# mlelarge/graph_neural_net

Hardware: AMD Instinct MI355X
Metric: graph-pairs/sec FGNN fwd+bwd, N=50 regular pairs (higher is better)
Workload: dtype f32

## Files before the change

graph_neural_net_amd/_lib.py:

```python
import ctypes as C
import os

import torch

_HERE = os.path.dirname(os.path.abspath(__file__))
LIB_PATH = os.environ.get('FGNN_LIB') or os.path.join(_HERE, 'libfgnn_hip.so')

FGNN_H = 32
FGNN_TILE = 32
FGNN_MAX_DEPTH = 3
FGNN_RANGE_WG = 256
FGNN_LSAP_MAX_N = 2048
FGNN_SCORE_SPLIT = 4

c_float_p = C.c_void_p


class Slab(C.Structure):
    _fields_ = [('ptr', C.c_void_p), ('gstride', C.c_longlong), ('ldp', C.c_longlong), ('C', C.c_int),
                ('nrm', C.c_void_p), ('beta', C.c_void_p)]


class MlpFwdArgs(C.Structure):
    _fields_ = [('G', C.c_int), ('N', C.c_int), ('depth', C.c_int), ('nmlp', C.c_int),
# ... 34 lines not shown
                ('dxb', C.c_void_p), ('dxb_gstride', C.c_longlong), ('dxb_ld', C.c_longlong),
                ('accumulate_dx', C.c_int), ('accumulate_dxb', C.c_int),
                ('wpart', C.c_void_p)]


class Mlp64PackJob(C.Structure):
    _fields_ = [('W', C.c_void_p * 3), ('bias', C.c_void_p * 3), ('cin', C.c_int), ('packed', C.c_void_p)]


class MlpBwdArgs(C.Structure):
    _fields_ = [('G', C.c_int), ('N', C.c_int), ('depth', C.c_int),
                ('nvalid', C.c_void_p),
                ('a', Slab), ('b', Slab),
                ('W', C.c_void_p * FGNN_MAX_DEPTH),
                ('bias', C.c_void_p * FGNN_MAX_DEPTH),
                ('dy', C.c_void_p), ('dgstride', C.c_longlong), ('ldd', C.c_longlong),
                ('z', C.c_void_p), ('zgstride', C.c_longlong), ('ldz', C.c_longlong),
                ('coef', C.c_void_p), ('s12', C.c_void_p), ('znrm', C.c_void_p),
                ('dxa', C.c_void_p), ('dxa_gstride', C.c_longlong), ('dxa_ld', C.c_longlong),
                ('dxb', C.c_void_p), ('dxb_gstride', C.c_longlong), ('dxb_ld', C.c_longlong),
                ('accumulate_a', C.c_int), ('accumulate_b', C.c_int),
                ('wpart', C.c_void_p), ('s12part', C.c_void_p), ('packed', C.c_void_p),
                ('s12tiles', C.c_void_p), ('s12_out', C.c_void_p), ('xbits', C.c_void_p), ('xdeg', C.c_void_p),
                ('ranges', C.c_void_p), ('cu_share', C.c_int)]


class Slab16(C.Structure):
    _fields_ = [('ptr', C.c_void_p), ('gstride', C.c_longlong), ('ldp', C.c_longlong), ('C', C.c_int),
                ('nrm', C.c_void_p), ('beta', C.c_void_p)]


class MlpFwd16Args(C.Structure):
    _fields_ = [('G', C.c_int), ('N', C.c_int), ('ldr', C.c_int), ('depth', C.c_int), ('nmlp', C.c_int),
                ('nvalid', C.c_void_p),
                ('a', Slab16), ('b', Slab16),
                ('z', C.c_void_p * 2), ('ldz', C.c_longlong),
                ('part', C.c_void_p * 2), ('cnt', C.c_void_p), ('packed', C.c_void_p), ('ranges', C.c_void_p)]


class MlpBwd16Args(C.Structure):
    _fields_ = [('G', C.c_int), ('N', C.c_int), ('ldr', C.c_int), ('depth', C.c_int),
                ('nvalid', C.c_void_p),
                ('a', Slab16), ('b', Slab16),
                ('dy', C.c_void_p), ('dgstride', C.c_longlong), ('ldd', C.c_longlong),
                ('z', C.c_void_p), ('zgstride', C.c_longlong), ('ldz', C.c_longlong),
                ('coef', C.c_void_p),
                ('dxa', C.c_void_p), ('dxa_gstride', C.c_longlong), ('dxa_ld', C.c_longlong),
# ... 70 lines not shown
    'fgnn_chan_matmul_fwd_fin_ord': [C.POINTER(Slab), C.POINTER(Slab), _VP, _VP, _VP, _VP, _VP, _F, _VP, _I, _I, _VP, _LL, _LL, _VP, _I, _VP],
    'fgnn_colmax_fwd': [C.POINTER(Slab), _VP, _I, _I, _VP, _VP, _VP],
    'fgnn_colmax_fwd_fin_supported': [_I],
    'fgnn_colmax_fwd_fin': [C.POINTER(Slab), _VP, _VP, _VP, _F, _VP, _I, _I, _VP, _VP, _VP],
    'fgnn_score_ce_fwd': [_VP, _VP, _VP, _I, _I, _I, _VP, _VP, _VP, _VP],
    'fgnn_score_row_blocks': [_I, _I],
    'fgnn_score_ce_fwd_blocks': [_VP, _VP, _VP, _I, _I, _I, _I, _VP, _VP, _VP, _VP],
    'fgnn_score_ce_bwd': [_VP, _VP, _VP, _VP, _VP, _VP, _I, _I, _I, _VP, _VP, _VP],
    'fgnn_inv_node_count': [_VP, _I, _VP, _VP],
    'fgnn_score_bwd': [_VP, _VP, _VP, _VP, _I, _I, _I, _VP, _VP, _VP],
    'fgnn_ce_fwd': [_VP, _VP, _I, _I, _VP, _VP, _VP],
    'fgnn_ce_bwd': [_VP, _VP, _VP, _VP, _I, _I, _VP, _VP],
    'fgnn_colmax_bwd': [_VP, _VP, _VP, _I, _I, _I, _VP, _LL, _LL, C.POINTER(Slab), _VP, _VP],
    'fgnn_gn_bwd_stats': [_VP, _LL, _LL, _VP, _LL, _LL, _VP, _VP, _I, _I, _I, _VP, _VP],
    'fgnn_gn_bwd_coef': [_VP, _VP, _VP, _I, _I, _I, _VP, _VP, _VP, _VP],
    'fgnn_gn_bwd_coef_tiles': [_VP, _VP, _VP, _I, _I, _I, _VP, _VP, _VP],
    'fgnn_grad_finalize': [_VP, _I, _I, _I, _I, _VP],
    'fgnn_gn_bwd_apply': [_VP, _LL, _LL, _VP, _LL, _LL, _VP, _VP, _I, _I, _I, _VP, _LL, _LL, _VP],
    'fgnn_mlp_bwd': [C.POINTER(MlpBwdArgs), _VP],
    'fgnn_mlp_bwd_x3': [C.POINTER(MlpBwdArgs), _VP],
    'fgnn_mlp_bwd_pair': [C.POINTER(MlpBwdArgs), C.POINTER(MlpBwdArgs), _VP],
    'fgnn_mlp_bwd_t16': [C.POINTER(MlpBwdArgs), _VP],
    'fgnn_mlp_bwd_t16_supported': [C.POINTER(MlpBwdArgs)],
    'fgnn_mlp_bwd_pair_t16': [C.POINTER(MlpBwdArgs), C.POINTER(MlpBwdArgs), _VP],
    'fgnn_mlp_bwd_pair_x3': [C.POINTER(MlpBwdArgs), C.POINTER(MlpBwdArgs), _VP],
    'fgnn_block1_struct_supported': [_I, _I, _I],
    'fgnn_block1_struct_table_floats': [_I],
    'fgnn_block1_struct_ws_floats': [_I, _I],
    'fgnn_block1_struct_rows': [_I, _I],
    'fgnn_block1_struct_fwd': [_VP, _VP, _I, _I, _VP, _VP, _VP, _VP, _VP, C.c_float, _VP, _VP, _VP, _LL, _LL, _VP, _VP, _VP, _VP, _VP, _VP, _VP],
    'fgnn_block1_struct_bwd': [_VP, _VP, _I, _I, _VP, _VP, _VP, _VP, _VP, _VP, _VP, _VP, _LL, _LL, _VP, _VP, _VP, _VP, _VP, _VP],
    'fgnn_block1_struct_fwd_pack': [_VP, _VP, _I, _I, _VP, _VP, _VP, _VP, _VP, C.c_float, _VP, _VP, _VP, _LL, _LL, _VP, _VP, _VP, _VP, _VP, _VP, _VP, _I, _VP],
    'fgnn_block1_struct_fwd16_pack': [_VP, _VP, _I, _I, _I, _VP, _VP, _VP, _VP, _VP, C.c_float, _VP, _VP, _VP, _LL, _LL, _VP, _VP, _VP, _VP, _VP, _VP, _VP, _I, _VP],
    'fgnn_block1_struct_fwd16': [_VP, _VP, _I, _I, _I, _VP, _VP, _VP, _VP, _VP, C.c_float, _VP, _VP, _VP, _LL, _LL, _VP, _VP, _VP, _VP, _VP, _VP, _VP],
    'fgnn_block1_struct_bwd16': [_VP, _VP, _I, _I, _I, _VP, _VP, _VP, _VP, _VP, _VP, _VP, _VP, _LL, _LL, _VP, _VP, _VP, _VP, _VP, _VP],
    'fgnn_mlp_bwd_coef_tiles_supported': [_I, _I],
    'fgnn_mlp_param_count': [_I, _I],
    'fgnn_reduce_partials': [_VP, _I, _I, _VP, _VP],
    'fgnn_chan_matmul_bwd': [C.POINTER(Slab), C.POINTER(Slab), _VP, _LL, _LL, _VP, _I, _I, _VP, _VP, _LL, _LL, _VP, _VP, _VP],
    'fgnn_chan_matmul_bwd_ord': [C.POINTER(Slab), C.POINTER(Slab), _VP, _LL, _LL, _VP, _I, _I, _VP, _VP, _LL, _LL, _VP, _VP, _VP, _I, _VP],
    'fgnn_sum_scale': [_VP, _I, _I, _F, _VP, _VP],
    'fgnn_adam_step': [_VP, _VP, _VP, _VP, _I, C.c_double, C.c_double, C.c_double, C.c_double, _I, C.c_double, _VP],
    'fgnn_adam_step_dev': [_VP, _VP, _VP, _VP, _I, _VP, _VP, _VP],
    'fgnn_expand_adjacency': [_VP, _VP, _I, _I, _VP, _VP],
    'fgnn_pack_adjacency': [_VP, _VP, _I, _I, _VP, _VP, _VP],
    'fgnn_pack_adjacency_ld': [_VP, _VP, _I, _I, _I, _VP, _VP, _VP],
# ... 123 lines not shown
```

graph_neural_net_amd/csrc/mlp_bwd_t16.hip:

```cpp
#include "fgnn_t16.h"
#include "fgnn_pack.h"

namespace {

using namespace t16;

constexpr int BWD_WG = 256;
constexpr int NW = 8;

DEVI float4 coef_from_sums(const float4 n, const float2 sv, float nv) {
    const float m = nv * nv;
    float4 k;
    k.x = n.x;
    k.y = n.y;
    k.z = m > 0.f ? -n.y * sv.y * n.w / m : 0.f;
    k.w = m > 0.f ? -n.y * sv.x / m : 0.f;
    return k;
}
DEVI int graph_nv(const rsrc_t &rnv, bool ragged, int g, int N) {
    const int v = __builtin_amdgcn_raw_buffer_load_b32(rnv, g * 4, 0, 0);
    return __builtin_amdgcn_readfirstlane(ragged ? v : N);
}

template <int CB>
struct Layout16 {
    static constexpr int DEPTH = 3;
    static constexpr PkBwd PK = pk_bwd(32, CB, DEPTH);
    static constexpr int OFF_W0A = PK.off_w1a, OFF_W0B = PK.off_w1b, OFF_W1 = PK.off_wh, OFF_WT1 = PK.off_wt, OFF_WT2 = PK.off_wt + 16;
    static constexpr int OFF_WT0A = PK.off_wt0a, OFF_WT0B = PK.off_wt0b;
    static constexpr int BIAS_F = PK.bias_f;
    static constexpr int WEIGHT_F = pk_pad_floats(PK.floats);
    static constexpr int NSLOT = 5;
    static constexpr int CIN = 32 + CB;
    static constexpr int PCOUNT = 32 * CIN + 32 + (DEPTH - 1) * (32 * 32 + 32);
    static constexpr int TILE_OFF = WEIGHT_F;
    static constexpr int REC_OFF = TILE_OFF + NW * NSLOT * TILE_F;
    static constexpr int WGK_OFF = REC_OFF + NW * 256;
    static constexpr int LIVE_OFF = WGK_OFF + FGNN_BWD_COEF_GRAPHS * 128;
    static constexpr int MAIN_F = LIVE_OFF + LIVE_LIST_CAP + NW;
    static constexpr int RED_F = NW * PCOUNT;
    static constexpr int LDS_F = MAIN_F > RED_F ? MAIN_F : RED_F;
};

template <int CB, bool PKD, bool SKIP, bool DXB>
__global__ __launch_bounds__(64 * NW, 2) void mlp_bwd_t16_kernel(const fgnn_mlp_bwd_args A, const int tpg, const int total_tiles) {
    extern __shared__ __attribute__((aligned(16))) float smem[];
    using L = Layout16<CB>;
    constexpr bool NB = CB == 32;
    const int lane = threadIdx.x & 63, wv = __builtin_amdgcn_readfirstlane(threadIdx.x >> 6);
    const int px = lane & 15, q = lane >> 4;
    const int P2 = A.N * A.N, hpg = 2 * tpg;
    const View va = make_view(A.a.ptr, A.a.gstride, A.a.ldp, A.G);
    const View vb = make_view(A.b.ptr, A.b.gstride, A.b.ldp, A.G);
    PackedSrc ps = {};
    if constexpr (PKD) ps = make_packed_src(A.xbits, A.xdeg, A.G, A.N);
    const View vdy = make_view(A.dy, A.dgstride, A.ldd, A.G);
    const View vz = make_view(A.z, A.zgstride, A.ldz, A.G);
    const View vdxa = make_view(A.dxa, A.dxa_gstride, A.dxa_ld, A.G);
    const View vdxb = make_view(A.dxb, A.dxb_gstride, A.dxb_ld, A.G);

    float *wl = smem;
    float *my = smem + L::TILE_OFF + wv * (L::NSLOT * TILE_F);
    float *XA = my, *XB = my + TILE_F, *S0 = my + 2 * TILE_F, *S1 = my + 3 * TILE_F, *S2 = my + 4 * TILE_F;
    const int lane_base = tile_lane_base(px, q);

    f32x4 dW0a[4], dW0b[4], dW1[4], dW2[4];
    float db0[2] = {0.f, 0.f}, db1[2] = {0.f, 0.f}, db2[2] = {0.f, 0.f}, dbx[2] = {0.f, 0.f};
#pragma unroll
    for (int k = 0; k < 4; ++k) dW0a[k] = dW0b[k] = dW1[k] = dW2[k] = zero4();

    const int nwg = gridDim.x;
    const int qq = total_tiles / nwg, rem = total_tiles % nwg;
    int T0 = blockIdx.x * qq + ((int)blockIdx.x < rem ? (int)blockIdx.x : rem);
    int T1 = T0 + qq + ((int)blockIdx.x < rem ? 1 : 0);
    if constexpr (SKIP) {
        T0 = A.ranges[blockIdx.x];
        T1 = A.ranges[blockIdx.x + 1];
    }
    const int H0 = 2 * T0, H1 = 2 * T1;
// ... 46 lines not shown
            while (h < H1) {
                const int g = h / hpg, hh = h - g * hpg;
                if (hh * 16 < P2) break;
                h += NW;
            }
            return __builtin_amdgcn_readfirstlane(h);
        }
    };

    pk_glds<NW>(smem, A.packed, L::WEIGHT_F, wv, lane);

    float mean[8], av[8], beta[8], kx[8], ky[8], kz[8], kw[8];
#pragma unroll
    for (int s = 0; s < 8; ++s) {
        mean[s] = 0.f;
        av[s] = 1.f;
        beta[s] = (NB && A.b.nrm && A.b.beta) ? A.b.beta[chan_s(s) + chan_q(q)] : 0.f;
        kx[s] = ky[s] = kz[s] = kw[s] = 0.f;
    }
    float4 *rec = reinterpret_cast<float4 *>(smem + L::REC_OFF) + wv * 64;
    auto fetch_records = [&](int g, int nv) {
        if (lane < 32) {
            float4 k4;
            if (from_tiles) k4 = wgK[(g - g0) * 32 + lane];
            else if (A.coef) k4 = reinterpret_cast<const float4 *>(A.coef)[(long long)g * FGNN_H + lane];
            else {
                const float4 n = reinterpret_cast<const float4 *>(A.znrm)[(long long)g * FGNN_H + lane];
                const float2 sv = reinterpret_cast<const float2 *>(A.s12)[(long long)g * FGNN_H + lane];
                k4 = coef_from_sums(n, sv, (float)nv);
            }
            rec[lane] = k4;
            if (NB && A.b.nrm) rec[32 + lane] = reinterpret_cast<const float4 *>(A.b.nrm)[(long long)g * A.b.C + lane];
        }
    };
    auto read_records = [&]() {
#pragma unroll
        for (int s = 0; s < 8; ++s) {
            const float4 k4 = rec[chan_s(s) + chan_q(q)];
            kx[s] = k4.x;
            ky[s] = k4.y;
            kz[s] = k4.z;
            kw[s] = k4.w;
            if (NB && A.b.nrm) {
                const float4 n = rec[32 + chan_s(s) + chan_q(q)];
                mean[s] = n.x;
                av[s] = n.y;
            }
        }
    };

    constexpr int NXB = CB == 32 ? 8 : 1;
    float xa[8], xb[NXB], dyr[8], zr[8];
    auto load_x = [&](int h) {
        const bool act = h < H1;
        const int g = __builtin_amdgcn_readfirstlane(act ? h / hpg : 0);
        const int p = (act ? h - g * hpg : 0) * 16 + px;
        const bool inb = act && p < P2;
        load8(xa, va, lane_voff(va, q, p, inb), g * va.gs4);
        if constexpr (CB == 32) {
            load8(xb, vb, lane_voff(vb, q, p, inb), g * vb.gs4);
        } else if constexpr (PKD) {
            int i, jj;
            row_col(p, A.N, rcpN, i, jj);
            const int ob = (inb && q == 0) ? (i * ps.words + (jj >> 5)) * 4 : OOB_OFF;
            const int od = (inb && q == 1 && i == jj) ? i * 4 : OOB_OFF;
            const unsigned w = (unsigned)__builtin_amdgcn_raw_buffer_load_b32(ps.bits, ob, g * ps.N * ps.words * 4, 0);
            const float d = __builtin_bit_cast(float, __builtin_amdgcn_raw_buffer_load_b32(ps.deg, od, g * ps.N * 4, 0));
            xb[0] = q == 0 ? (((w >> (jj & 31)) & 1u) ? 1.f : 0.f) : d;
        } else {
            xb[0] = buf_load(vb, (inb && q < 2) ? q * vb.ld4 + 4 * p : OOB_OFF, g * vb.gs4);
        }
    };
    auto load_dyz = [&](int h) {
        const bool act = h < H1;
        const int g = __builtin_amdgcn_readfirstlane(act ? h / hpg : 0);
        const int p = (act ? h - g * hpg : 0) * 16 + px;
        const bool inb = act && p < P2;
        load8(dyr, vdy, lane_voff(vdy, q, p, inb), g * vdy.gs4);
        load8(zr, vz, lane_voff(vz, q, p, inb), g * vz.gs4);
    };

    int h = next_half(SKIP ? H0 : H0 + wv);
    load_x(h);
    int cached_g = -1, cur_nv = A.N;

    if (from_tiles) {
        const int g1 = T1 > T0 ? (T1 - 1) / tpg : g0 - 1;
        float2 *scr = reinterpret_cast<float2 *>(smem + L::TILE_OFF);
        const int cc = threadIdx.x & 31, sl = threadIdx.x >> 5;
        for (int g = g0; g <= g1; ++g) {
            float p1 = 0.f, p2 = 0.f;
            constexpr int TS = (64 * NW) / 32, U = 8;
            for (int t0 = sl; t0 < tpg; t0 += TS * U) {
                float2 v[U];
#pragma unroll
                for (int k = 0; k < U; ++k) {
                    const int t = t0 + TS * k;
                    v[k] = reinterpret_cast<const float2 *>(A.s12tiles)[((long long)g * tpg + (t < tpg ? t : 0)) * FGNN_H + cc];
                }
#pragma unroll
                for (int k = 0; k < U; ++k) {
                    if (t0 + TS * k < tpg) {
                        p1 += v[k].x;
                        p2 += v[k].y;
                    }
                }
            }
            scr[sl * 32 + cc] = make_float2(p1, p2);
            __syncthreads();
            if (threadIdx.x < 32) {
                float s1 = 0.f, s2 = 0.f;
#pragma unroll
                for (int k = 0; k < (64 * NW) / 32; ++k) {
                    s1 += scr[k * 32 + cc].x;
                    s2 += scr[k * 32 + cc].y;
                }
                const float2 sv = make_float2(s1, s2);
                if (A.s12_out) reinterpret_cast<float2 *>(A.s12_out)[(long long)g * FGNN_H + cc] = sv;
                const float4 n = reinterpret_cast<const float4 *>(A.znrm)[(long long)g * FGNN_H + cc];
                wgK[(g - g0) * 32 + cc] = coef_from_sums(n, sv, (float)graph_nv(rnv, ragged, g, A.N));
            }
            __syncthreads();
        }
    }
    if (h < H1) {
        const int g = h / hpg;
        cur_nv = graph_nv(rnv, ragged, g, A.N);
        fetch_records(g, cur_nv);
        cached_g = g;
    }
    if constexpr (CB == 2) {
        for (int e = lane; e < 16 * TLD; e += 64) XB[e] = 0.f;
    }
    __syncthreads();
    load_dyz(h);
    if (cached_g >= 0) read_records();

    while (h < H1) {
        const int hn = next_half(SKIP ? h + 1 : h + NW);
        const int g = __builtin_amdgcn_readfirstlane(h / hpg), hh = h - g * hpg;
        const int p = hh * 16 + px;
        const bool inb = p < P2;
        if (g != cached_g) {
            cur_nv = graph_nv(rnv, ragged, g, A.N);
            fetch_records(g, cur_nv);
            read_records();
// ... 18 lines not shown
            }
            stage8(XA, lane_base, xa);
            if constexpr (CB == 32) {
                stage8(XB, lane_base, yb);
            } else {
                if (q < 2) XB[8 * q * TLD + px] = yb[0];
            }
            f32x4 acc[2];
            load_bias(acc, wl + L::BIAS_F, 0, q);
            gemm32<L::OFF_W0A>(acc, wl, xa, lane);
            if constexpr (CB == 32) gemm32<L::OFF_W0B>(acc, wl, yb, lane);
            else gemm2<L::OFF_W0B>(acc, wl, q < 2 ? yb[0] : 0.f, lane);
            load_x(hn);
#pragma unroll
            for (int s = 0; s < 8; ++s) h1[s] = relu1(acc[s >> 2][s & 3]);
            stage8(S0, lane_base, h1);
            load_bias(acc, wl + L::BIAS_F, 1, q);
            gemm32<L::OFF_W1>(acc, wl, h1, lane);
#pragma unroll
            for (int s = 0; s < 8; ++s) h2[s] = relu1(acc[s >> 2][s & 3]);
            stage8(S1, lane_base, h2);
        }
        float dpre[8];
#pragma unroll
        for (int s = 0; s < 8; ++s) dpre[s] = fmaf(kz[s], zr[s] - kx[s], fmaf(ky[s], dyr[s], kw[s]));
        if (!full) {
#pragma unroll
            for (int s = 0; s < 8; ++s) dpre[s] = valid ? dpre[s] : 0.f;
        }
        stage8(S2, lane_base, dpre);
        load_dyz(hn);
        __builtin_amdgcn_sched_barrier(0);
        {
            f32x4 a2[2];
            a2[0] = a2[1] = zero4();
            gemm32<L::OFF_WT2>(a2, wl, dpre, lane);
            wgrad16(dW2, db2, S2, S1, lane);
#pragma unroll
            for (int s = 0; s < 8; ++s) dpre[s] = h2[s] > 0.f ? a2[s >> 2][s & 3] : 0.f;
        }
        __builtin_amdgcn_sched_barrier(0);
        stage8(S1, lane_base, dpre);
        {
            f32x4 a2[2];
            a2[0] = a2[1] = zero4();
            gemm32<L::OFF_WT1>(a2, wl, dpre, lane);
// ... 76 lines not shown
            red[32 * CIN + 32 + 1024 + c1] = db1[1];
            red[32 * CIN + 32 + 1056 + 1024 + c0] = db2[0];
            red[32 * CIN + 32 + 1056 + 1024 + c1] = db2[1];
        }
    }
    __syncthreads();
    static_assert(PCOUNT % 4 == 0, "partials are summed four at a time");
    float4 *out = reinterpret_cast<float4 *>(A.wpart + (long long)blockIdx.x * PCOUNT);
    const float4 *part4 = reinterpret_cast<const float4 *>(smem);
    for (int e = threadIdx.x; e < PCOUNT / 4; e += 64 * NW) {
        float4 a = part4[e];
#pragma unroll
        for (int w = 1; w < NW; ++w) {
            const float4 b = part4[w * (PCOUNT / 4) + e];
            a.x += b.x;
            a.y += b.y;
            a.z += b.z;
            a.w += b.w;
        }
        out[e] = a;
    }
}

template <int CB, bool PKD, bool SKIP, bool DXB>
int launch16(const fgnn_mlp_bwd_args *a, int tpg, int total, hipStream_t st) {
    constexpr int LDS = Layout16<CB>::LDS_F * 4;
    static_assert(LDS <= 160 * 1024, "LDS budget");
    static LdsAttrCache attr_cache;
    (void)fgnn_raise_lds(attr_cache, (const void *)mlp_bwd_t16_kernel<CB, PKD, SKIP, DXB>, LDS);
    hipLaunchKernelGGL((mlp_bwd_t16_kernel<CB, PKD, SKIP, DXB>), dim3(a->cu_share == 2 && !SKIP ? BWD_WG / 2 : BWD_WG), dim3(64 * NW), LDS, st, *a,
                       tpg, total);
    FGNN_LAUNCH_CHECK();
    return 0;
}
template <int CB, bool PKD, bool DXB>
int launch16s(const fgnn_mlp_bwd_args *a, int tpg, int total, hipStream_t st) {
    return a->ranges ? launch16<CB, PKD, true, DXB>(a, tpg, total, st) : launch16<CB, PKD, false, DXB>(a, tpg, total, st);
}

}

extern "C" int fgnn_mlp_bwd_t16_supported(const fgnn_mlp_bwd_args *a) {
    if (!a || a->depth != 3 || a->a.C != 32 || a->a.nrm || !a->dxa || a->accumulate_a || a->accumulate_b || !a->packed || a->N > 256) return 0;
    if (a->b.C == 32) return (a->b.nrm && a->dxb && !a->xbits) ? 1 : 0;
    if (a->b.C == 2) return (!a->b.nrm && !a->dxb) ? 1 : 0;
    return 0;
}

extern "C" int fgnn_mlp_bwd_t16(const fgnn_mlp_bwd_args *a, void *stream) {
    FGNN_CHECK(a != nullptr, "fgnn_mlp_bwd_t16: null args");
    FGNN_CHECK(fgnn_mlp_bwd_t16_supported(a), "fgnn_mlp_bwd_t16: built for depth 3, slab a = 32 raw channels with dx stored, slab b = 32 normalised "
               "channels with dx stored or 2 raw channels without dx, an operand image of kind 5, N <= 256; use fgnn_mlp_bwd");
    FGNN_CHECK(a->G > 0 && a->N > 0 && a->a.ptr && (a->b.ptr || (a->xbits && a->b.C == 2)), "fgnn_mlp_bwd_t16: bad G / N / slabs");
    FGNN_CHECK(!a->xbits || a->xdeg, "fgnn_mlp_bwd_t16: xbits without xdeg (fgnn_adjacency_degree)");
    FGNN_CHECK(a->dy && a->z && a->wpart, "fgnn_mlp_bwd_t16: missing dy/z/wpart");
    FGNN_CHECK(a->coef || (a->s12 && a->znrm) || (a->s12tiles && a->znrm), "fgnn_mlp_bwd_t16: need coef, or s12 + znrm, or s12tiles + znrm");
    FGNN_CHECK(BWD_WG == fgnn_mlp_bwd_num_workgroups() && BWD_WG == FGNN_RANGE_WG, "fgnn_mlp_bwd_t16: workgroup count differs from fgnn_mlp_bwd");
    {
        const long long lim = 0x7fffffffll / 4, G = a->G;
        FGNN_CHECK(G * a->a.gstride < lim && G * a->b.gstride < lim && G * a->dgstride < lim && G * a->zgstride < lim &&
                   G * a->dxa_gstride < lim && G * a->dxb_gstride < lim,
                   "fgnn_mlp_bwd_t16: a tensor exceeds 2 GiB (32-bit buffer addressing); split the batch");
    }
    for (int l = 0; l < a->depth; ++l) FGNN_CHECK(a->W[l] && a->bias[l], "fgnn_mlp_bwd_t16: missing weights layer %d", l);
    const int tpg = fgnn_tiles_per_graph(a->N);
    const long long total = (long long)a->G * tpg;
    FGNN_CHECK(total < (1ll << 29), "fgnn_mlp_bwd_t16: too many tiles");
    FGNN_CHECK(!a->ranges || (a->nvalid && !a->s12tiles), "fgnn_mlp_bwd_t16: ranges need nvalid and exclude s12tiles");
    FGNN_CHECK(!a->s12tiles || fgnn_mlp_bwd_coef_tiles_supported(a->G, a->N), "fgnn_mlp_bwd_t16: s12tiles needs a workgroup's tile range to span <= %d graphs",
               FGNN_BWD_COEF_GRAPHS);
    hipStream_t st = (hipStream_t)stream;
    if (a->b.C == 32) return launch16s<32, false, true>(a, tpg, (int)total, st);
    if (a->xbits) return launch16s<2, true, false>(a, tpg, (int)total, st);
    return launch16s<2, false, false>(a, tpg, (int)total, st);
}
```

graph_neural_net_amd/engine.py:

```python
import ctypes as C
import os

import torch

from . import _lib

EPS = 1e-05


class ParamLayout:

    def __init__(self, original_features_num=2, num_blocks=4, in_features=32, out_features=32, depth_of_mlp=3):
        if in_features != _lib.FGNN_H or out_features != _lib.FGNN_H:
            raise RuntimeError('the fused engine is built for in_features = out_features = 32 (got %d, %d); other widths '
                               'run through the per-layer modules (layers.MlpBlock_Real)' % (in_features, out_features))
        if not 1 <= depth_of_mlp <= _lib.FGNN_MAX_DEPTH:
            raise RuntimeError('depth_of_mlp must be in 1..%d' % _lib.FGNN_MAX_DEPTH)
        if original_features_num not in (2, 32):
            raise RuntimeError('the fused engine is built for original_features_num = 2 or 32 (got %d); other widths run '
                               'through the per-layer modules (layers.MlpBlock_Real)' % original_features_num)
        self.c0 = original_features_num
        self.num_blocks = num_blocks
        self.depth = depth_of_mlp
        self.entries = []
# ... 91 lines not shown

    def keys(self):
        return list(self._items)

    def clear(self):
        self._items.clear()

    def __len__(self):
        return len(self._items)

    def __iter__(self):
        return iter(list(self._items))

    def values(self):
        return [e for e, _ in self._items.values()]


class FgnnEngine:
    SKIP_PADDING_TILES = True
    MM_ORDER = True
    PAIR_BWD = os.environ.get('FGNN_PAIR_BWD', '1') != '0'
    PACK_IN_STRUCT = os.environ.get('FGNN_PACK_IN_STRUCT', '1') != '0'
    T16 = os.environ.get('FGNN_T16', 'pair,bwd')

    MFMA = os.environ.get('FGNN_MFMA', 'f32')

    BLOCK1 = os.environ.get('FGNN_BLOCK1', 'generic')

    def __init__(self, layout, G, N, device, ragged=False, cu_share=0, mfma=None, block1=None):
        _lib.load()
        self.T16 = type(self).T16
        self.cu_share = int(cu_share)
        mfma = self.MFMA if mfma is None else mfma
        if mfma not in ('f32', 'x3'):
            raise ValueError("mfma must be 'f32' or 'x3' (got %r)" % (mfma,))
        self.x3 = (mfma == 'x3' and not ragged and layout.depth == 3 and layout.c0 in (2, 32))
        block1 = self.BLOCK1 if block1 is None else block1
        if block1 not in ('generic', 'structured'):
            raise ValueError("block1 must be 'generic' or 'structured' (got %r)" % (block1,))
        self.struct1 = (block1 == 'structured' and cu_share == 0
                        and bool(_lib.load().fgnn_block1_struct_supported(N, layout.depth, layout.c0)))
        self._struct = None
        self.decisions = None
        self.layout = layout
        self.G, self.N = G, N
        self.P = N * N
# ... 284 lines not shown
        if self.cu_share == 2 and self.ranges is None:
            nwg //= 2
        L = self.layout
        keys = [(k, j) for k in range(1, L.num_blocks + 1) for j in (1, 2, 3)]
        self._bwd = {
            'dE': torch.empty(self.G, 32, self.N, **f32),
            'dy': [act(), act()],
            'dmult': act(), 'dy1': act(), 'dy2': act(),
            's12': {kj: torch.empty(self.G * 32 * 2, **f32) for kj in keys},
            'wpart': {kj: torch.empty(nwg * L.mlp[kj]['count'], **f32)
                      for kj in keys},
            's12part': torch.empty(self.G * self.tpg * 32 * 2, **f32),
            'coef': [torch.empty(self.G * 32 * 4, **f32) for _ in range(3)],
            'nwg': nwg,
            'gscale': torch.empty(1, **f32),
        }
        return self._bwd

    def _coef(self, kj, slot):
        W = self._bwd
        _lib.call('fgnn_gn_bwd_coef', _lib.ptr(W['s12'][kj]), _lib.ptr(self.nrm[kj]), self._nv(), self.G, 32, self.N,
                  _lib.ptr(W['coef'][slot]), None, None, _lib.stream_ptr())

    def _mlp_bwd(self, params, k, j, a, b, dy, coef, dxa, dxb, acc_a, acc_b, emit=False, dx_strides=None):
        args = self._mlp_bwd_args(params, k, j, a, b, dy, coef, dxa, dxb, acc_a, acc_b, emit, dx_strides)
        entry = 'fgnn_mlp_bwd_x3' if (self.x3 and j != 3) else 'fgnn_mlp_bwd'
        if j == 3 and b is not None and self._t16_bwd3(b.C) and _lib.load().fgnn_mlp_bwd_t16_supported(C.byref(args)):
            entry = 'fgnn_mlp_bwd_t16'
        elif self._packs[('b', k, j)][0] == 5:
            args.packed = None
        _lib.call(entry, C.byref(args), _lib.stream_ptr(),
                  tag='mlp_bwd[cin=%d,dx=%d]' % (a.C + (b.C if b is not None else 0),
                                                (a.C if dxa is not None else 0) + (b.C if (b is not None and dxb is not None) else 0)))

    def _mlp_bwd_pair(self, params, k, sin, din, emit):
        W = self._bwd
        a1 = self._mlp_bwd_args(params, k, 1, sin, None, W['dy1'], None, None, None, False, False, False, None)
        a2 = self._mlp_bwd_args(params, k, 2, sin, None, W['dy2'], None, din, None, True, False, emit, None)
        entry = 'fgnn_mlp_bwd_pair_x3' if self.x3 else ('fgnn_mlp_bwd_pair_t16' if self._t16_pair(sin.C) else 'fgnn_mlp_bwd_pair')
        _lib.call(entry, C.byref(a1), C.byref(a2), _lib.stream_ptr(),
                  tag='mlp_bwd_pair[cin=%d,dx=%d]' % (sin.C, sin.C if din is not None else 0))

    def _mlp_bwd_args(self, params, k, j, a, b, dy, coef, dxa, dxb, acc_a, acc_b, emit, dx_strides):
        L = self.layout
        W = self._bwd
        rec = L.mlp[(k, j)]
        gs = 32 * self.ldp
        args = _lib.MlpBwdArgs()
        args.G, args.N, args.depth = self.G, self.N, L.depth
        args.nvalid = self.nvalid.data_ptr() if self.nvalid is not None else None
        args.a = a
        if b is not None:
            args.b = b
        for l in range(L.depth):
            args.W[l] = self._w(params, rec['w'][l])
            args.bias[l] = self._w(params, rec['b'][l])
        args.dy, args.dgstride, args.ldd = dy.data_ptr(), gs, self.ldp
        args.z, args.zgstride, args.ldz = self.z[(k, j)].data_ptr(), gs, self.ldp
        if isinstance(coef, str):
            args.s12tiles = W['s12part'].data_ptr()
            args.s12_out = W['s12'][(k, j)].data_ptr()
            args.znrm = self.nrm[(k, j)].data_ptr()
        elif coef is not None:
            args.coef = coef.data_ptr()
        else:
            args.s12 = W['s12'][(k, j)].data_ptr()
            args.znrm = self.nrm[(k, j)].data_ptr()
        dgs, dld = (gs, self.ldp) if dx_strides is None else dx_strides
        if dxa is not None:
            args.dxa, args.dxa_gstride, args.dxa_ld = dxa.data_ptr(), (gs if (b is not None and dx_strides is not None) else dgs), \
                (self.ldp if (b is not None and dx_strides is not None) else dld)
        if dxb is not None:
            args.dxb, args.dxb_gstride, args.dxb_ld = dxb.data_ptr(), dgs, dld
        args.accumulate_a, args.accumulate_b = int(acc_a), int(acc_b)
        args.wpart = W['wpart'][(k, j)].data_ptr()
        args.packed = self._packs[('b', k, j)][4].data_ptr()
        self._packed_input(args, k)
        if self.ranges is not None:
            args.ranges = self.ranges.data_ptr()
        args.cu_share = self.cu_share
        if emit:
            args.s12part = W['s12part'].data_ptr()
# ... 7 lines not shown
        if gscale_dev is not None:
            gs_t = gscale_dev
        else:
            self._set_gscale(grad_scale / self.total_nodes)
        e1, e2 = self.E[:B], self.E[B:]
        _lib.call('fgnn_score_ce_bwd', _lib.ptr(e1), _lib.ptr(e2), _lib.ptr(self.scores), _lib.ptr(self.lse),
                  self._nv(), _lib.ptr(gs_t), B, 32, N, _lib.ptr(W['dE'][:B]), _lib.ptr(W['dE'][B:]), st)
        return self.backward_from_dE(params, grads, W['dE'], finalize=finalize)

    def _set_gscale(self, gs):
        W = self._bwd
        if W.get('gscale_value') != gs:
            W['gscale'].fill_(gs)
            W['gscale_value'] = gs

    def backward_from_dE(self, params, grads, dE, finalize=True, dx=None):
        L = self.layout
        W = self._alloc_bwd()
        st = _lib.stream_ptr()
        gs = 32 * self.ldp
        K = L.num_blocks
        in_prologue = bool(_lib.load().fgnn_mlp_bwd_coef_tiles_supported(self.G, self.N)) and self.ranges is None
        dy = W['dy'][0]
        out = self._slab_z(K, 3, params)
        _lib.call('fgnn_colmax_bwd', _lib.ptr(dE), _lib.ptr(self.idx), self._nv(), self.G, 32, self.N,
                  _lib.ptr(dy), gs, self.ldp, C.byref(out), _lib.ptr(W['s12'][(K, 3)]), st)
        for k in range(K, 0, -1):
            sin = self._slab_in(k, params)
            first = (k == 1)
            din = None if first else W['dy'][(K - k + 1) % 2]
            dxs = None
            if first and dx is not None:
                if self.xbits is not None or self.x3 or tuple(dx.shape) != (self.G, L.c0, self.N, self.N) or dx.dtype != torch.float32 \
                        or not dx.is_contiguous():
                    raise RuntimeError('FgnnEngine: the input gradient needs a dense fp32 input, the fp32-MFMA kernels (mfma="f32") '
                                       'and a contiguous (G, c0, N, N) fp32 dx')
                din, dxs = dx, (L.c0 * self.P, self.P)
            self._mlp_bwd(params, k, 3, self._slab_raw(self.mult[k]), sin, dy,
                          None if k == K else ('tiles' if in_prologue else W['coef'][2]), W['dmult'], din, False, False, dx_strides=dxs)
            if first and self.struct1 and self.xbits is not None and dxs is None:
                self._struct_bwd(params)
                dy = din
                continue
            ya, yb = self._slab_z(k, 1, params), self._slab_z(k, 2, params)
            _lib.call('fgnn_chan_matmul_bwd_ord', C.byref(ya), C.byref(yb), _lib.ptr(W['dmult']), gs, self.ldp,
                      self._nv(), self.G, self.N, _lib.ptr(W['dy1']), _lib.ptr(W['dy2']), gs, self.ldp,
                      _lib.ptr(W['s12'][(k, 1)]), _lib.ptr(W['s12'][(k, 2)]),
                      _lib.ptr(self.mm_order) if self.mm_order is not None else None, self._fill(), st, tag='fgnn_chan_matmul_bwd')
            if first:
                W['struct_rows'] = 0
            if self.PAIR_BWD and dxs is None and L.depth == 3 and sin.C in (2, 32):
                self._mlp_bwd_pair(params, k, sin, din, emit=not first)
            else:
                self._mlp_bwd(params, k, 1, sin, None, W['dy1'], None, din, None, True, False, dx_strides=dxs)
                self._mlp_bwd(params, k, 2, sin, None, W['dy2'], None, din, None, True, False, emit=not first, dx_strides=dxs)
            if not first and not in_prologue:
                _lib.call('fgnn_gn_bwd_coef_tiles', _lib.ptr(W['s12part']), _lib.ptr(self.nrm[(k - 1, 3)]), self._nv(),
                          self.G, 32, self.N, _lib.ptr(W['s12'][(k - 1, 3)]), _lib.ptr(W['coef'][2]), st)
            dy = din
        if finalize:
            self.grad_finalize(grads)
        return grads
# ... 87 lines not shown
```

include/fgnn_hip.h:

```cpp
#ifndef FGNN_HIP_H
#define FGNN_HIP_H

#ifdef __cplusplus
extern "C" {
#endif

#define FGNN_H 32
#define FGNN_TILE 32
#define FGNN_MAX_DEPTH 3

typedef struct {
    const float *ptr;
    long long gstride;
    long long ldp;
    int C;
    const float *nrm;
    const float *beta;
} fgnn_slab;

const char *fgnn_last_error(void);
int fgnn_version(void);
int fgnn_tiles_per_graph(int N);
int fgnn_mlp_bwd_num_workgroups(void);

// ... 177 lines not shown
typedef struct {
    int G, N, depth;
    const int *nvalid;
    fgnn_slab a, b;
    const float *W[FGNN_MAX_DEPTH];
    const float *bias[FGNN_MAX_DEPTH];
    const float *dy;  long long dgstride, ldd;
    const float *z;   long long zgstride, ldz;
    const float *coef;
    const float *s12;
    const float *znrm;
    float *dxa; long long dxa_gstride, dxa_ld;
    float *dxb; long long dxb_gstride, dxb_ld;
    int accumulate_a, accumulate_b;
    float *wpart;
    float *s12part;
    const float *packed;
    const float *s12tiles;
    float *s12_out;
    const unsigned *xbits;
    const float *xdeg;
    const int *ranges;
    int cu_share;
} fgnn_mlp_bwd_args;
int fgnn_mlp_bwd(const fgnn_mlp_bwd_args *args, void *stream);
int fgnn_mlp_bwd_x3(const fgnn_mlp_bwd_args *args, void *stream);
int fgnn_mlp_bwd_pair(const fgnn_mlp_bwd_args *m1, const fgnn_mlp_bwd_args *m2, void *stream);
int fgnn_mlp_bwd_pair_x3(const fgnn_mlp_bwd_args *m1, const fgnn_mlp_bwd_args *m2, void *stream);
int fgnn_mlp_bwd_t16_supported(const fgnn_mlp_bwd_args *args);
int fgnn_mlp_bwd_t16(const fgnn_mlp_bwd_args *args, void *stream);
int fgnn_mlp_bwd_pair_t16(const fgnn_mlp_bwd_args *m1, const fgnn_mlp_bwd_args *m2, void *stream);
#define FGNN_BWD_COEF_GRAPHS 4
int fgnn_mlp_bwd_coef_tiles_supported(int G, int N);
int fgnn_mlp_param_count(int Cin, int depth);
int fgnn_reduce_partials(const float *wpart, int num_wg, int count, float *out, void *stream);

#define FGNN_MAX_GRAD_JOBS 16
typedef struct {
    const float *wpart; int count; float *out;
    const float *s12; const float *nrm; float *dgn_w; float *dgn_b;
    int rows;
    float scale;
    const float *scale_dev;
} fgnn_grad_job;
int fgnn_grad_finalize(const fgnn_grad_job *jobs, int njobs, int num_wg, int G, int C, void *stream);
int fgnn_inv_node_count(const int *nvalid, int B, float *out, void *stream);

int fgnn_chan_matmul_bwd(const fgnn_slab *ya, const fgnn_slab *yb, const float *dm, long long dmgstride, long long ldm,
                         const int *nvalid, int G, int N,
                         float *da, float *db, long long ogstride, long long ldo,
                         float *s12a ,
                         float *s12b , void *stream);
// ... 171 lines not shown
```

Baseline: 42520.

## Fuse column-max backward into t16 MLP backward via virtual sparse dy

```diff
diff --git a/graph_neural_net_amd/_lib.py b/graph_neural_net_amd/_lib.py
--- a/graph_neural_net_amd/_lib.py
+++ b/graph_neural_net_amd/_lib.py
@@ -80,7 +80,8 @@
                 ('accumulate_a', C.c_int), ('accumulate_b', C.c_int),
                 ('wpart', C.c_void_p), ('s12part', C.c_void_p), ('packed', C.c_void_p),
                 ('s12tiles', C.c_void_p), ('s12_out', C.c_void_p), ('xbits', C.c_void_p), ('xdeg', C.c_void_p),
-                ('ranges', C.c_void_p), ('cu_share', C.c_int)]
+                ('ranges', C.c_void_p), ('cu_share', C.c_int),
+                ('de', C.c_void_p), ('deidx', C.c_void_p)]
 
 
 class Slab16(C.Structure):
@@ -197,6 +198,7 @@
     'fgnn_mlp_bwd_pair': [C.POINTER(MlpBwdArgs), C.POINTER(MlpBwdArgs), _VP],
     'fgnn_mlp_bwd_t16': [C.POINTER(MlpBwdArgs), _VP],
     'fgnn_mlp_bwd_t16_supported': [C.POINTER(MlpBwdArgs)],
+    'fgnn_mlp_bwd_t16_vdy_supported': [C.POINTER(MlpBwdArgs)],
     'fgnn_mlp_bwd_pair_t16': [C.POINTER(MlpBwdArgs), C.POINTER(MlpBwdArgs), _VP],
     'fgnn_mlp_bwd_pair_x3': [C.POINTER(MlpBwdArgs), C.POINTER(MlpBwdArgs), _VP],
     'fgnn_block1_struct_supported': [_I, _I, _I],
diff --git a/graph_neural_net_amd/csrc/mlp_bwd_t16.hip b/graph_neural_net_amd/csrc/mlp_bwd_t16.hip
--- a/graph_neural_net_amd/csrc/mlp_bwd_t16.hip
+++ b/graph_neural_net_amd/csrc/mlp_bwd_t16.hip
@@ -42,7 +42,7 @@
     static constexpr int LDS_F = MAIN_F > RED_F ? MAIN_F : RED_F;
 };
 
-template <int CB, bool PKD, bool SKIP, bool DXB>
+template <int CB, bool PKD, bool SKIP, bool DXB, bool VDY = false>
 __global__ __launch_bounds__(64 * NW, 2) void mlp_bwd_t16_kernel(const fgnn_mlp_bwd_args A, const int tpg, const int total_tiles) {
     extern __shared__ __attribute__((aligned(16))) float smem[];
     using L = Layout16<CB>;
@@ -55,6 +55,8 @@
     PackedSrc ps = {};
     if constexpr (PKD) ps = make_packed_src(A.xbits, A.xdeg, A.G, A.N);
     const View vdy = make_view(A.dy, A.dgstride, A.ldd, A.G);
+    const View vde = make_view(A.de, 32ll * A.N, A.N, VDY ? A.G : 0);
+    const View vdi = make_view(reinterpret_cast<const float *>(A.deidx), 32ll * A.N, A.N, VDY ? A.G : 0);
     const View vz = make_view(A.z, A.zgstride, A.ldz, A.G);
     const View vdxa = make_view(A.dxa, A.dxa_gstride, A.dxa_ld, A.G);
     const View vdxb = make_view(A.dxb, A.dxb_gstride, A.dxb_ld, A.G);
@@ -147,7 +149,11 @@
     auto fetch_records = [&](int g, int nv) {
         if (lane < 32) {
             float4 k4;
-            if (from_tiles) k4 = wgK[(g - g0) * 32 + lane];
+            if (VDY && g - g0 >= FGNN_BWD_COEF_GRAPHS) {
+                const float4 n = reinterpret_cast<const float4 *>(A.znrm)[(long long)g * FGNN_H + lane];
+                const float2 sv = reinterpret_cast<const float2 *>(A.s12_out)[(long long)g * FGNN_H + lane];
+                k4 = coef_from_sums(n, sv, (float)nv);
+            } else if (VDY || from_tiles) k4 = wgK[(g - g0) * 32 + lane];
             else if (A.coef) k4 = reinterpret_cast<const float4 *>(A.coef)[(long long)g * FGNN_H + lane];
             else {
                 const float4 n = reinterpret_cast<const float4 *>(A.znrm)[(long long)g * FGNN_H + lane];
@@ -176,6 +182,7 @@
 
     constexpr int NXB = CB == 32 ? 8 : 1;
     float xa[8], xb[NXB], dyr[8], zr[8];
+    int dix[VDY ? 8 : 1];
     auto load_x = [&](int h) {
         const bool act = h < H1;
         const int g = __builtin_amdgcn_readfirstlane(act ? h / hpg : 0);
@@ -201,7 +208,16 @@
         const int g = __builtin_amdgcn_readfirstlane(act ? h / hpg : 0);
         const int p = (act ? h - g * hpg : 0) * 16 + px;
         const bool inb = act && p < P2;
-        load8(dyr, vdy, lane_voff(vdy, q, p, inb), g * vdy.gs4);
+        if constexpr (VDY) {
+            int i, jj;
+            row_col(p, A.N, rcpN, i, jj);
+            const int vo = inb ? chan_q(q) * vde.ld4 + 4 * i : OOB_OFF;
+            load8(dyr, vde, vo, g * vde.gs4);
+#pragma unroll
+            for (int s = 0; s < 8; ++s) dix[s] = __builtin_amdgcn_raw_buffer_load_b32(vdi.r, vo, g * vdi.gs4 + chan_s(s) * vdi.ld4, 0);
+        } else {
+            load8(dyr, vdy, lane_voff(vdy, q, p, inb), g * vdy.gs4);
+        }
         load8(zr, vz, lane_voff(vz, q, p, inb), g * vz.gs4);
     };
 
@@ -247,6 +263,86 @@
             }
             __syncthreads();
         }
+    }
+    if constexpr (VDY) {
+        const int g1 = T1 > T0 ? (T1 - 1) / tpg : g0 - 1;
+        constexpr int U = 8;
+        const int nchunk = (A.N + 63) >> 6;
+        for (int ga = g0; ga <= g1; ga += 2) {
+            const bool two = ga < g1;
+            const int la = __builtin_amdgcn_raw_buffer_load_b32(rnv, ga * 4, 0, 0), lb = __builtin_amdgcn_raw_buffer_load_b32(rnv, (two ? ga + 1 : ga) * 4, 0, 0);
+            const int nva = ragged ? la : A.N, nvb = ragged ? lb : A.N;
+            float4 n[U];
+#pragma unroll
+            for (int k = 0; k < U; ++k)
+                n[k] = reinterpret_cast<const float4 *>(A.znrm)[(long long)(k < 4 || !two ? ga : ga + 1) * FGNN_H + wv + NW * (k & 3)];
+            float lo1[U], hi1[U], lo2[U], hi2[U], t1[U], t2[U];
+#pragma unroll
+            for (int k = 0; k < U; ++k) lo1[k] = hi1[k] = lo2[k] = hi2[k] = t1[k] = t2[k] = 0.f;
+            for (int ck = 0; ck < nchunk; ++ck) {
+                const int i = 64 * ck + lane;
+                float d[U], zv[U];
+                int bi[U];
+#pragma unroll
+                for (int k = 0; k < U; ++k) {
+                    const int g = k < 4 ? ga : ga + 1, c = wv + NW * (k & 3);
+                    const int vo = (i < A.N && (k < 4 || two)) ? c * vde.ld4 + 4 * i : OOB_OFF;
+                    d[k] = buf_load(vde, vo, g * vde.gs4);
+                    bi[k] = __builtin_amdgcn_raw_buffer_load_b32(vdi.r, vo, g * vdi.gs4, 0);
+                }
+#pragma unroll
+                for (int k = 0; k < U; ++k) {
+                    const int g = k < 4 ? ga : ga + 1, c = wv + NW * (k & 3);
+                    const bool in = i < A.N && (k < 4 || two) && (unsigned)bi[k] < (unsigned)A.N;
+                    zv[k] = buf_load(vz, in ? c * vz.ld4 + 4 * (i * A.N + bi[k]) : OOB_OFF, g * vz.gs4);
+                }
+                int na = la, nb = lb;
+                asm volatile("" : "+v"(na), "+v"(nb));
+                na = ragged ? na : A.N;
+                nb = ragged ? nb : A.N;
+#pragma unroll
+                for (int k = 0; k < U; ++k) {
+                    const bool ok = i < (k < 4 ? na : nb);
+                    float s1 = 0.f, s2 = 0.f;
+                    if (ok) {
+                        s1 += d[k];
+                        s2 += d[k] * (zv[k] - n[k].x);
+                    }
+                    s1 = wave_sum(s1);
+                    s2 = wave_sum(s2);
+                    if (ck & 1) {
+                        if (ck == 1) {
+                            lo1[k] = t1[k] + s1;
+                            lo2[k] = t2[k] + s2;
+                        } else {
+                            hi1[k] = t1[k] + s1;
+                            hi2[k] = t2[k] + s2;
+                        }
+                        t1[k] = t2[k] = 0.f;
+                    } else {
+                        t1[k] = s1;
+                        t2[k] = s2;
+                    }
+                }
+            }
+#pragma unroll
+            for (int k = 0; k < U; ++k) {
+                if (nchunk == 1) {
+                    lo1[k] = t1[k];
+                    lo2[k] = t2[k];
+                } else if (nchunk == 3) {
+                    hi1[k] = t1[k];
+                    hi2[k] = t2[k];
+                }
+                if ((k < 4 || two) && lane == 0) {
+                    const int g = k < 4 ? ga : ga + 1, c = wv + NW * (k & 3);
+                    const float2 sv = make_float2(lo1[k] + hi1[k], lo2[k] + hi2[k]);
+                    reinterpret_cast<float2 *>(A.s12_out)[(long long)g * FGNN_H + c] = sv;
+                    if (g - g0 < FGNN_BWD_COEF_GRAPHS) wgK[(g - g0) * 32 + c] = coef_from_sums(n[k], sv, (float)(k < 4 ? nva : nvb));
+                }
+            }
+        }
+        __syncthreads();
     }
     if (h < H1) {
         const int g = h / hpg;
@@ -311,6 +407,12 @@
             stage8(S1, lane_base, h2);
         }
         float dpre[8];
+        if constexpr (VDY) {
+            int i, jj;
+            row_col(p, A.N, rcpN, i, jj);
+#pragma unroll
+            for (int s = 0; s < 8; ++s) dyr[s] = jj == dix[s] ? dyr[s] : 0.f;
+        }
 #pragma unroll
         for (int s = 0; s < 8; ++s) dpre[s] = fmaf(kz[s], zr[s] - kx[s], fmaf(ky[s], dyr[s], kw[s]));
         if (!full) {
@@ -433,44 +535,53 @@
     }
 }
 
-template <int CB, bool PKD, bool SKIP, bool DXB>
+template <int CB, bool PKD, bool SKIP, bool DXB, bool VDY>
 int launch16(const fgnn_mlp_bwd_args *a, int tpg, int total, hipStream_t st) {
     constexpr int LDS = Layout16<CB>::LDS_F * 4;
     static_assert(LDS <= 160 * 1024, "LDS budget");
     static LdsAttrCache attr_cache;
-    (void)fgnn_raise_lds(attr_cache, (const void *)mlp_bwd_t16_kernel<CB, PKD, SKIP, DXB>, LDS);
-    hipLaunchKernelGGL((mlp_bwd_t16_kernel<CB, PKD, SKIP, DXB>), dim3(a->cu_share == 2 && !SKIP ? BWD_WG / 2 : BWD_WG), dim3(64 * NW), LDS, st, *a,
-                       tpg, total);
+    (void)fgnn_raise_lds(attr_cache, (const void *)mlp_bwd_t16_kernel<CB, PKD, SKIP, DXB, VDY>, LDS);
+    hipLaunchKernelGGL((mlp_bwd_t16_kernel<CB, PKD, SKIP, DXB, VDY>), dim3(a->cu_share == 2 && !SKIP ? BWD_WG / 2 : BWD_WG), dim3(64 * NW), LDS,
+                       st, *a, tpg, total);
     FGNN_LAUNCH_CHECK();
     return 0;
 }
-template <int CB, bool PKD, bool DXB>
+template <int CB, bool PKD, bool DXB, bool VDY = false>
 int launch16s(const fgnn_mlp_bwd_args *a, int tpg, int total, hipStream_t st) {
-    return a->ranges ? launch16<CB, PKD, true, DXB>(a, tpg, total, st) : launch16<CB, PKD, false, DXB>(a, tpg, total, st);
+    return a->ranges ? launch16<CB, PKD, true, DXB, VDY>(a, tpg, total, st) : launch16<CB, PKD, false, DXB, VDY>(a, tpg, total, st);
 }
 
 }
 
 extern "C" int fgnn_mlp_bwd_t16_supported(const fgnn_mlp_bwd_args *a) {
+    if (a && (a->de || a->deidx)) return fgnn_mlp_bwd_t16_vdy_supported(a);
     if (!a || a->depth != 3 || a->a.C != 32 || a->a.nrm || !a->dxa || a->accumulate_a || a->accumulate_b || !a->packed || a->N > 256) return 0;
     if (a->b.C == 32) return (a->b.nrm && a->dxb && !a->xbits) ? 1 : 0;
     if (a->b.C == 2) return (!a->b.nrm && !a->dxb) ? 1 : 0;
     return 0;
 }
 
+extern "C" int fgnn_mlp_bwd_t16_vdy_supported(const fgnn_mlp_bwd_args *a) {
+    if (!a || !a->de || !a->deidx || !a->znrm || !a->s12_out || a->coef || a->s12 || a->s12tiles) return 0;
+    if (a->depth != 3 || a->a.C != 32 || a->a.nrm || !a->dxa || a->accumulate_a || a->accumulate_b || !a->packed || a->N > 256) return 0;
+    return (a->b.C == 32 && a->b.nrm && a->dxb && !a->xbits) ? 1 : 0;
+}
+
 extern "C" int fgnn_mlp_bwd_t16(const fgnn_mlp_bwd_args *a, void *stream) {
     FGNN_CHECK(a != nullptr, "fgnn_mlp_bwd_t16: null args");
     FGNN_CHECK(fgnn_mlp_bwd_t16_supported(a), "fgnn_mlp_bwd_t16: built for depth 3, slab a = 32 raw channels with dx stored, slab b = 32 normalised "
-               "channels with dx stored or 2 raw channels without dx, an operand image of kind 5, N <= 256; use fgnn_mlp_bwd");
+               "channels with dx stored or 2 raw channels without dx, an operand image of kind 5, N <= 256; use fgnn_mlp_bwd (with de / deidx: see "
+               "fgnn_mlp_bwd_t16_vdy_supported)");
     FGNN_CHECK(a->G > 0 && a->N > 0 && a->a.ptr && (a->b.ptr || (a->xbits && a->b.C == 2)), "fgnn_mlp_bwd_t16: bad G / N / slabs");
     FGNN_CHECK(!a->xbits || a->xdeg, "fgnn_mlp_bwd_t16: xbits without xdeg (fgnn_adjacency_degree)");
-    FGNN_CHECK(a->dy && a->z && a->wpart, "fgnn_mlp_bwd_t16: missing dy/z/wpart");
-    FGNN_CHECK(a->coef || (a->s12 && a->znrm) || (a->s12tiles && a->znrm), "fgnn_mlp_bwd_t16: need coef, or s12 + znrm, or s12tiles + znrm");
+    const bool vdy = a->de || a->deidx;
+    FGNN_CHECK((vdy || a->dy) && a->z && a->wpart, "fgnn_mlp_bwd_t16: missing dy/z/wpart");
+    FGNN_CHECK(vdy || a->coef || (a->s12 && a->znrm) || (a->s12tiles && a->znrm), "fgnn_mlp_bwd_t16: need coef, or s12 + znrm, or s12tiles + znrm");
     FGNN_CHECK(BWD_WG == fgnn_mlp_bwd_num_workgroups() && BWD_WG == FGNN_RANGE_WG, "fgnn_mlp_bwd_t16: workgroup count differs from fgnn_mlp_bwd");
     {
         const long long lim = 0x7fffffffll / 4, G = a->G;
         FGNN_CHECK(G * a->a.gstride < lim && G * a->b.gstride < lim && G * a->dgstride < lim && G * a->zgstride < lim &&
-                   G * a->dxa_gstride < lim && G * a->dxb_gstride < lim,
+                   G * a->dxa_gstride < lim && G * a->dxb_gstride < lim && G * 32 * a->N < lim,
                    "fgnn_mlp_bwd_t16: a tensor exceeds 2 GiB (32-bit buffer addressing); split the batch");
     }
     for (int l = 0; l < a->depth; ++l) FGNN_CHECK(a->W[l] && a->bias[l], "fgnn_mlp_bwd_t16: missing weights layer %d", l);
@@ -481,6 +592,7 @@
     FGNN_CHECK(!a->s12tiles || fgnn_mlp_bwd_coef_tiles_supported(a->G, a->N), "fgnn_mlp_bwd_t16: s12tiles needs a workgroup's tile range to span <= %d graphs",
                FGNN_BWD_COEF_GRAPHS);
     hipStream_t st = (hipStream_t)stream;
+    if (vdy) return launch16s<32, false, true, true>(a, tpg, (int)total, st);
     if (a->b.C == 32) return launch16s<32, false, true>(a, tpg, (int)total, st);
     if (a->xbits) return launch16s<2, true, false>(a, tpg, (int)total, st);
     return launch16s<2, false, false>(a, tpg, (int)total, st);
diff --git a/graph_neural_net_amd/engine.py b/graph_neural_net_amd/engine.py
--- a/graph_neural_net_amd/engine.py
+++ b/graph_neural_net_amd/engine.py
@@ -137,6 +137,7 @@
     PAIR_BWD = os.environ.get('FGNN_PAIR_BWD', '1') != '0'
     PACK_IN_STRUCT = os.environ.get('FGNN_PACK_IN_STRUCT', '1') != '0'
     T16 = os.environ.get('FGNN_T16', 'pair,bwd')
+    VIRTUAL_DY = os.environ.get('FGNN_VIRTUAL_DY', '1') != '0'
 
     MFMA = os.environ.get('FGNN_MFMA', 'f32')
 
@@ -467,6 +468,16 @@
         _lib.call('fgnn_gn_bwd_coef', _lib.ptr(W['s12'][kj]), _lib.ptr(self.nrm[kj]), self._nv(), self.G, 32, self.N,
                   _lib.ptr(W['coef'][slot]), None, None, _lib.stream_ptr())
 
+    def _mlp_bwd_virtual_dy(self, params, k, a, b, dE, dxa, dxb):
+        if not (self.VIRTUAL_DY and b is not None and self._t16_bwd3(b.C)):
+            return False
+        args = self._mlp_bwd_args(params, k, 3, a, b, None, 'virtual', dxa, dxb, False, False, False, None)
+        args.de, args.deidx = dE.data_ptr(), self.idx.data_ptr()
+        if not _lib.load().fgnn_mlp_bwd_t16_vdy_supported(C.byref(args)):
+            return False
+        _lib.call('fgnn_mlp_bwd_t16', C.byref(args), _lib.stream_ptr(), tag='mlp_bwd[cin=%d,dx=%d]' % (a.C + b.C, a.C + b.C))
+        return True
+
     def _mlp_bwd(self, params, k, j, a, b, dy, coef, dxa, dxb, acc_a, acc_b, emit=False, dx_strides=None):
         args = self._mlp_bwd_args(params, k, j, a, b, dy, coef, dxa, dxb, acc_a, acc_b, emit, dx_strides)
         entry = 'fgnn_mlp_bwd_x3' if (self.x3 and j != 3) else 'fgnn_mlp_bwd'
@@ -500,9 +511,12 @@
         for l in range(L.depth):
             args.W[l] = self._w(params, rec['w'][l])
             args.bias[l] = self._w(params, rec['b'][l])
-        args.dy, args.dgstride, args.ldd = dy.data_ptr(), gs, self.ldp
+        args.dy, args.dgstride, args.ldd = (dy.data_ptr() if dy is not None else None), gs, self.ldp
         args.z, args.zgstride, args.ldz = self.z[(k, j)].data_ptr(), gs, self.ldp
-        if isinstance(coef, str):
+        if coef == 'virtual':
+            args.s12_out = W['s12'][(k, j)].data_ptr()
+            args.znrm = self.nrm[(k, j)].data_ptr()
+        elif isinstance(coef, str):
             args.s12tiles = W['s12part'].data_ptr()
             args.s12_out = W['s12'][(k, j)].data_ptr()
             args.znrm = self.nrm[(k, j)].data_ptr()
@@ -556,9 +570,6 @@
         K = L.num_blocks
         in_prologue = bool(_lib.load().fgnn_mlp_bwd_coef_tiles_supported(self.G, self.N)) and self.ranges is None
         dy = W['dy'][0]
-        out = self._slab_z(K, 3, params)
-        _lib.call('fgnn_colmax_bwd', _lib.ptr(dE), _lib.ptr(self.idx), self._nv(), self.G, 32, self.N,
-                  _lib.ptr(dy), gs, self.ldp, C.byref(out), _lib.ptr(W['s12'][(K, 3)]), st)
         for k in range(K, 0, -1):
             sin = self._slab_in(k, params)
             first = (k == 1)
@@ -570,8 +581,15 @@
                     raise RuntimeError('FgnnEngine: the input gradient needs a dense fp32 input, the fp32-MFMA kernels (mfma="f32") '
                                        'and a contiguous (G, c0, N, N) fp32 dx')
                 din, dxs = dx, (L.c0 * self.P, self.P)
-            self._mlp_bwd(params, k, 3, self._slab_raw(self.mult[k]), sin, dy,
-                          None if k == K else ('tiles' if in_prologue else W['coef'][2]), W['dmult'], din, False, False, dx_strides=dxs)
+            if k == K and dx is None and self._mlp_bwd_virtual_dy(params, k, self._slab_raw(self.mult[k]), sin, dE, W['dmult'], din):
+                pass
+            else:
+                if k == K:
+                    out = self._slab_z(K, 3, params)
+                    _lib.call('fgnn_colmax_bwd', _lib.ptr(dE), _lib.ptr(self.idx), self._nv(), self.G, 32, self.N,
+                              _lib.ptr(dy), gs, self.ldp, C.byref(out), _lib.ptr(W['s12'][(K, 3)]), st)
+                self._mlp_bwd(params, k, 3, self._slab_raw(self.mult[k]), sin, dy,
+                              None if k == K else ('tiles' if in_prologue else W['coef'][2]), W['dmult'], din, False, False, dx_strides=dxs)
             if first and self.struct1 and self.xbits is not None and dxs is None:
                 self._struct_bwd(params)
                 dy = din
diff --git a/include/fgnn_hip.h b/include/fgnn_hip.h
--- a/include/fgnn_hip.h
+++ b/include/fgnn_hip.h
@@ -223,12 +223,15 @@
     const float *xdeg;
     const int *ranges;
     int cu_share;
+    const float *de;
+    const int *deidx;
 } fgnn_mlp_bwd_args;
 int fgnn_mlp_bwd(const fgnn_mlp_bwd_args *args, void *stream);
 int fgnn_mlp_bwd_x3(const fgnn_mlp_bwd_args *args, void *stream);
 int fgnn_mlp_bwd_pair(const fgnn_mlp_bwd_args *m1, const fgnn_mlp_bwd_args *m2, void *stream);
 int fgnn_mlp_bwd_pair_x3(const fgnn_mlp_bwd_args *m1, const fgnn_mlp_bwd_args *m2, void *stream);
 int fgnn_mlp_bwd_t16_supported(const fgnn_mlp_bwd_args *args);
+int fgnn_mlp_bwd_t16_vdy_supported(const fgnn_mlp_bwd_args *args);
 int fgnn_mlp_bwd_t16(const fgnn_mlp_bwd_args *args, void *stream);
 int fgnn_mlp_bwd_pair_t16(const fgnn_mlp_bwd_args *m1, const fgnn_mlp_bwd_args *m2, void *stream);
 #define FGNN_BWD_COEF_GRAPHS 4
```

After: 42360 (median of 2 runs). Within noise of the previous version (-0.4%).
